# can-lehmann/exprgrad

Measured on AMD Instinct MI355X. Metric: GFLOP/s matmul 4096^3 f32 (1 GPU), higher is better.
Workload: dtype f32

## Files before the change

exprgrad_amd/csrc/kernels/gemm_f32_mfma.hip:

```cpp
#include "gemm_skinny.hpp"
#include "gemm_f32_pair.hpp"
#include "gemm_fused.hpp"
#include "gemm_layout.hpp"
#include "gemm_plan.hpp"

#include <algorithm>
#include <cstdio>
#include <cstdlib>
#include <cstring>
#include <string>
#include <type_traits>

#include "../eg_internal.hpp"

namespace {

using namespace eg::gemm;

inline bool aligned16(const void* p) { return (reinterpret_cast<uintptr_t>(p) & 15) == 0; }

const GemmSwitches& gemm_switches() {
  thread_local GemmSwitches s;
  thread_local unsigned seen = 0;
  const unsigned gen = eg::sw::generation();
// ... 119 lines not shown
  if (lane == 0) {
    float* c = C + m * ldc + n;
    float v = s;
    if (accumulate) v = *c + v;
    if (bias) v = v + bias[n];
    *c = v;
  }
}

__global__ __launch_bounds__(256) void gemm_small_kernel(const float* __restrict__ A, const float* __restrict__ B, float* C,
                                                         const float* __restrict__ bias, long M, long N, long K,
                                                         long a_sm, long a_sk, long b_sk, long b_sn, long ldc,
                                                         int accumulate) {
  gemm_small_body(blockIdx.x, A, B, C, bias, M, N, K, a_sm, a_sk, b_sk, b_sn, ldc, accumulate);
}

__global__ __launch_bounds__(256) void gemm_small_pair_kernel(eg::SmallGemm g0, eg::SmallGemm g1, long blocks0) {
  const bool second = (long)blockIdx.x >= blocks0;
  const eg::SmallGemm& g = second ? g1 : g0;
  gemm_small_body(second ? (long)blockIdx.x - blocks0 : (long)blockIdx.x, g.A, g.B, g.C, g.bias, g.M, g.N, g.K, g.a_sm, g.a_sk, g.b_sk,
                  g.b_sn, g.ldc, g.accumulate);
}

int run_gemm(eg_ctx* ctx, const GemmProblem& pr, GemmArgs args, const GemmSwitches& sw) {
  if (!args.ones_row) args.a_rows = args.M;
  const GemmPlan p = plan_gemm(pr, sw);
  const bool a_kc = pr.a_kc, b_kc = pr.b_kc;
  if (p.route == Route::Remainder) {
    for (int i = 0; i < p.nparts; ++i) {
      const auto& c = p.parts[i];
      GemmArgs part = args;
      part.A = args.A + c.row0 * (a_kc ? args.lda : 1);
      part.B = args.B + c.col0 * (b_kc ? args.ldb : 1);
      part.C = args.C + c.row0 * args.ldc + c.col0;
      if (args.bias) part.bias = args.bias + c.col0;
      part.M = part.a_rows = c.M;
      part.N = c.N;
      const int rc = run_gemm(ctx, problem_of(ctx, part, a_kc, b_kc, pr.conv, pr.vec_ok, pr.a_vec_only, true), part, sw);
      if (rc) return rc;
    }
    return EG_OK;
  }
  args.tiles_m = p.tiles_m;
  args.tiles_n = p.tiles_n;
  args.splits = p.splits;
  args.k_per_split = p.k_per_split;
  args.edge_splits = p.edge_splits;
  args.k_per_split_edge = p.k_per_split_edge;
  args.tail_tiles = p.tail_tiles;
  args.tail_splits = p.tail_splits;
  args.tail_k_per_split = p.tail_k_per_split;
  args.x_rows = p.x_rows;
  args.wide_store = p.wide_store;
  args.nt_store = p.nt_store;
  args.no_skew = p.no_skew;
  args.prio = p.prio && ctx->on_side_lane;
  float* scratch = nullptr;
  if (p.workspace_floats > 0) {
    const long scratch_floats = p.second == Second::Tree ? eg::colsum_scratch_floats(ctx, p.splits, args.M * args.N) : 0;
    const int rc = eg::ensure_workspace(ctx, (size_t)(p.workspace_floats + scratch_floats) * sizeof(float));
    if (rc) return rc;
    args.partial = static_cast<float*>(ctx->workspace);
    scratch = args.partial + p.workspace_floats;
  }
  const dim3 grid((unsigned)p.grid), block(p.block);
  const hipStream_t s = ctx->stream;
  switch (p.route) {
    case Route::Small:
      hipLaunchKernelGGL(gemm_small_kernel, grid, block, 0, s, args.A, args.B, args.C, args.bias, args.M, args.N, args.K,
                         a_kc ? args.lda : 1, a_kc ? 1 : args.lda, b_kc ? 1 : args.ldb, b_kc ? args.ldb : 1, args.ldc, args.accumulate);
      break;
    case Route::Skinny:
      hipLaunchKernelGGL((eg_skinny::gemm_skinny_nn_kernel<4>), grid, block, (size_t)args.K * 64, s, args.A, args.B, args.C, args.bias,
                         args.M, (int)args.N, (int)args.K, args.lda, args.ldb, args.ldc, args.accumulate);
      break;
    case Route::ExtraRows:
      if (sw.trace) args.trace = trace_begin(ctx, grid.x, 8);
      hipLaunchKernelGGL((gemm_f32_mfma_kernel<256, 256, BK, 128, 64, 1, false, false, 4, true, 0, 0, true, true>), grid, block, 0, s, args);
      EG_HIP_CHECK(hipGetLastError());
// ... 64 lines not shown

namespace eg {
namespace gemm {
const GemmSwitches& current_switches() { return gemm_switches(); }

int sgemm_exact(eg_ctx* ctx, int trans_a, int trans_b, long M, long N, long K, const float* A, long lda, const float* B, long ldb,
                float* C, long ldc, int accumulate, const float* bias, const unsigned* run_if, unsigned run_if_val) {
  EG_REQUIRE(ctx, EG_ERR_INVALID, "eg_sgemm: ctx is NULL");
  EG_REQUIRE(M >= 0 && N >= 0 && K >= 0, EG_ERR_INVALID, "eg_sgemm: negative extent");
  if (M == 0 || N == 0) return EG_OK;
  EG_REQUIRE(C, EG_ERR_INVALID, "eg_sgemm: C is NULL");
  EG_REQUIRE(K == 0 || (A && B), EG_ERR_INVALID, "eg_sgemm: NULL operand");
  EG_REQUIRE(lda >= (trans_a ? M : K) && ldb >= (trans_b ? K : N) && ldc >= N, EG_ERR_INVALID,
             "eg_sgemm: leading dimension smaller than the row length");
  int rc = eg::set_device(ctx);
  if (rc) return rc;

  GemmArgs args = sgemm_args(M, N, K, A, lda, B, ldb, C, ldc, accumulate, bias);
  args.run_if = run_if;
  args.run_if_val = run_if_val;
  return run_gemm(ctx, sgemm_problem(ctx, args, !trans_a, trans_b != 0), args, gemm_switches());
}

bool exact_single_launch(eg_ctx* ctx, int trans_a, int trans_b, long M, long N, long K, const float* A, long lda, const float* B,
                         long ldb, const float* C, long ldc, const float* bias) {
  const GemmArgs args = sgemm_args(M, N, K, A, lda, B, ldb, const_cast<float*>(C), ldc, 0, bias);
  return exact_single_launch(plan_gemm(sgemm_problem(ctx, args, !trans_a, trans_b != 0), gemm_switches()));
}
}
}

extern "C" int eg_sgemm(eg_ctx* ctx, int trans_a, int trans_b, int64_t M, int64_t N, int64_t K, const float* A,
                        int64_t lda, const float* B, int64_t ldb, float* C, int64_t ldc, int accumulate,
                        const float* bias) {
  const int rc = eg::gemm::sgemm_split(ctx, trans_a, trans_b, M, N, K, A, lda, B, ldb, C, ldc, accumulate, bias);
  if (rc != EG_ERR_UNSUPPORTED) return rc;
  return eg::gemm::sgemm_exact(ctx, trans_a, trans_b, M, N, K, A, lda, B, ldb, C, ldc, accumulate, bias);
}

namespace eg {
namespace gemm {
bool ones_row_supported(int trans_a, int trans_b, long M, long N, long K, const float* A, long lda, const float* B, long ldb) {
  const bool vec_a = operand_vec(lda, trans_a ? M : K, aligned16(A)), vec_b = operand_vec(ldb, trans_b ? K : N, aligned16(B));
  const char* off = eg::sw::raw("EG_NO_ONES_ROW");
  return vec_a && vec_b && K >= 16 && !((M + 1) * N <= 16384 && K <= 2048) && !(off && off[0] && off[0] != '0');
}

int sgemm_ones_row(eg_ctx* ctx, int trans_a, int trans_b, long M, long N, long K, const float* A, long lda, const float* B,
                   long ldb, float* C, long ldc, int accumulate) {
  EG_REQUIRE(ctx, EG_ERR_INVALID, "sgemm_ones_row: ctx is NULL");
// ... 402 lines not shown
```

exprgrad_amd/csrc/kernels/gemm_f32_mfma.hpp:

```cpp
#ifndef __HIPCC_RTC__
#pragma once
#include <hip/hip_runtime.h>
#endif

namespace eg {
namespace gemm {

typedef float f32x16 __attribute__((ext_vector_type(16)));
typedef float f32x4 __attribute__((ext_vector_type(4)));

struct GemmArgs {
  const float* A;
  const float* B;
  float* C;
  const float* bias;
  float* partial;
  long M, N, K;
  long lda, ldb, ldc;
  long k_per_split;
  int tiles_m, tiles_n;
  int accumulate;
  int splits;
  int edge_splits;
  long k_per_split_edge;
// ... 997 lines not shown
    const float* arow = park + (mb * 16 + r) * PS + 4 * g + kh * (BN / 2);
    const float* brow = w2s + ((g * 16 + r) << 2) + kh * (BN / 2) * 16;
    rd4 d0 = {0.f, 0.f, 0.f, 0.f}, d1 = {0.f, 0.f, 0.f, 0.f}, d2 = {0.f, 0.f, 0.f, 0.f}, d3 = {0.f, 0.f, 0.f, 0.f};
#pragma unroll
    for (int s2 = 0; s2 < BN / 32; s2 += 2) {
      const rd4 a0 = *reinterpret_cast<const rd4*>(arow + 16 * s2);
      const rd4 b0 = *reinterpret_cast<const rd4*>(brow + 256 * s2);
      const rd4 a1 = *reinterpret_cast<const rd4*>(arow + 16 * s2 + 16);
      const rd4 b1 = *reinterpret_cast<const rd4*>(brow + 256 * s2 + 256);
#pragma unroll
      for (int j = 0; j < 4; j += 2) {
        d0 = __builtin_amdgcn_mfma_f32_16x16x4f32(a0[j], b0[j], d0, 0, 0, 0);
        d1 = __builtin_amdgcn_mfma_f32_16x16x4f32(a1[j], b1[j], d1, 0, 0, 0);
        d2 = __builtin_amdgcn_mfma_f32_16x16x4f32(a0[j + 1], b0[j + 1], d2, 0, 0, 0);
        d3 = __builtin_amdgcn_mfma_f32_16x16x4f32(a1[j + 1], b1[j + 1], d3, 0, 0, 0);
      }
    }
#pragma unroll
    for (int v = 0; v < 4; ++v) half[v] = (d0[v] + d2[v]) + (d1[v] + d3[v]);
    if (kh == 1) *reinterpret_cast<rd4*>(rdx + (mb * 64 + lane) * 4) = rd4{half[0], half[1], half[2], half[3]};
  }
};

template <int BM, int BN, int BK, int WM, int WN, bool A_KC, bool B_KC, int VEC, bool EDGE, int CONV, int ABL, bool DMA,
          class Epi, bool XR = false>
__device__ __forceinline__ void gemm_block_at(const GemmArgs& a, const int block_id) {
  constexpr int WAVES = Geometry<BM, BN, WM, WN>::WAVES, WAVES_N = BN / WN;
  constexpr int MI = WM / 32, NI = WN / 32;
  constexpr int SA = LdsStride<BM, BK, A_KC>::value, SB = LdsStride<BN, BK, B_KC>::value;

  constexpr bool RD = Epi::RD_N > 0;
  constexpr int RD_FLOATS = RD ? 2 * (BM / WM) * 32 * (BN + 4) + BN * 16 + 4 * 64 * 4 : 0;
  constexpr int OPERAND_FLOATS = 2 * BK * (SA + SB) + (XR ? 2 * BK * 32 : 0);
  __shared__ __attribute__((aligned(16))) float lds[RD_FLOATS > OPERAND_FLOATS ? RD_FLOATS : OPERAND_FLOATS];

  const int tid = threadIdx.x;
  const int lane = tid & 63;
  const int wave = tid >> 6;
  const int wm0 = (wave / WAVES_N) * WM;
  const int wn0 = (wave % WAVES_N) * WN;
  if (a.run_if && *(volatile const unsigned*)a.run_if != a.run_if_val) return;
  if (a.prio) __builtin_amdgcn_s_setprio(3);
  trace_stamp<WAVES>(a, wave, lane, 0);

  const WorkItem w = decode_work<BM, BN>(a, block_id);
  const long m_blk = w.m_blk, n_blk = w.n_blk;
  const long k_begin = (long)w.split * w.k_slice;
  const long k_end = min(a.K, k_begin + w.k_slice);

  f32x16 acc[MI][NI];
  zero_acc(acc);
  if constexpr (RD) stage_row_product_weights<Epi, BM, BN, WM, WN>(a, lds, n_blk, tid);
  trace_stamp<WAVES>(a, wave, lane, 1);
  const bool il = run_k_loop<BM, BN, BK, WM, WN, A_KC, B_KC, VEC, EDGE, CONV, ABL, DMA, XR>(a, lds, acc, w, k_begin, k_end, tid, wm0, wn0);

  if constexpr ((ABL & 128) != 0) {
    float s = 0.f;
// ... 172 lines not shown
        }
      } else if (accumulate) {
#pragma unroll
        for (int r = 0; r < 16; ++r) {
          const long m = m_base + RS * acc_reg_row(r);
          if (m >= a.M || !n_ok) continue;
          col[m * ldo] = (col[m * ldo] + acc[i][j][r]) + bias;
        }
      } else {
#pragma unroll
        for (int r = 0; r < 16; ++r) {
          const long m = m_base + RS * acc_reg_row(r);
          if (m >= a.M || !n_ok) continue;
          col[m * ldo] = acc[i][j][r] + bias;
        }
      }
    }
  }
  trace_stamp<WAVES>(a, wave, lane, 3);
}

template <int BM, int BN, int BK, int WM, int WN, bool A_KC, bool B_KC, int VEC, bool EDGE, int CONV, int ABL, bool DMA,
          class Epi, bool XR = false>
__device__ __forceinline__ void gemm_block(const GemmArgs& a) {
  gemm_block_at<BM, BN, BK, WM, WN, A_KC, B_KC, VEC, EDGE, CONV, ABL, DMA, Epi, XR>(a, (int)blockIdx.x);
}

template <int BM, int BN, int WM, int WN, int MINB, bool EDGE, int VEC>
struct WavesPerSimd {
  static constexpr int plain = (MINB * Geometry<BM, BN, WM, WN>::WAVES + 3) / 4;
  static constexpr int value = (EDGE && VEC == 1 && BM * BN >= 128 * 64 && plain > 2) ? 2
                               : (EDGE && BN == 64 && BM >= 128 && plain == 4)        ? 3
                                                                                       : plain;
};

template <int BM, int BN, int BK, int WM, int WN, int MINB, bool A_KC, bool B_KC, int VEC, bool EDGE, int CONV,
          int ABL = 0, bool DMA = false, bool XR = false>
__global__ __launch_bounds__((Geometry<BM, BN, WM, WN>::NT), (WavesPerSimd<BM, BN, WM, WN, MINB, EDGE, VEC>::value)) void
gemm_f32_mfma_kernel(GemmArgs a) {
  gemm_block<BM, BN, BK, WM, WN, A_KC, B_KC, VEC, EDGE, CONV, ABL, DMA, EpiNone, XR>(a);
}

template <int BK, bool A_KC, bool B_KC>
__global__ __launch_bounds__(256, 4) void gemm_streamk_kernel(GemmArgs a) {
  constexpr int BM = 64, BN = 64, WM = 32, WN = 32;
  constexpr int SA = LdsStride<BM, BK, A_KC>::value, SB = LdsStride<BN, BK, B_KC>::value;
// ... 242 lines not shown
```

exprgrad_amd/csrc/kernels/gemm_fused.hpp:

```cpp
#pragma once
#include <string>

#include "../eg_internal.hpp"

namespace eg {
namespace gemm {

struct FusedLaunch {
  int bm = 0, bn = 0, bk = 0, wm = 0, wn = 0, minb = 0, nt = 0;
  bool a_kc = false, b_kc = false, edge = false, dma = false;
  int vec = 1;
  int splits = 1;
  unsigned grid = 0;
  bool narrow = false;
  int narrow_k = 0;
  unsigned narrow_grid = 0;
  long matrix_k_per_split = 0;
  alignas(8) unsigned char args[336];
  unsigned args_size = 0;
  unsigned waves = 0;
};
constexpr int MAX_EPILOGUE_OPERANDS = 6;

int plan_fused(eg_ctx* ctx, int trans_a, int trans_b, long M, long N, long K, const float* A, long lda, const float* B,
               long ldb, float* C, long ldc, const float* bias, FusedLaunch& out);

int sgemm_exact(eg_ctx* ctx, int trans_a, int trans_b, long M, long N, long K, const float* A, long lda, const float* B, long ldb,
                float* C, long ldc, int accumulate, const float* bias, const unsigned* run_if = nullptr, unsigned run_if_val = 0);
bool exact_single_launch(eg_ctx* ctx, int trans_a, int trans_b, long M, long N, long K, const float* A, long lda, const float* B,
                         long ldb, const float* C, long ldc, const float* bias);
int sgemm_split(eg_ctx* ctx, int trans_a, int trans_b, long M, long N, long K, const float* A, long lda, const float* B, long ldb,
                float* C, long ldc, int accumulate, const float* bias);

int sgemm_batched(eg_ctx* ctx, int trans_a, int trans_b, long batch, long M, long N, long K, const float* A, long lda, long stride_a,
                  const float* B, long ldb, long stride_b, float* C, long ldc, long stride_c, int accumulate, const float* bias);
int dgemm(eg_ctx* ctx, int trans_a, int trans_b, long M, long N, long K, const double* A, long lda, const double* B, long ldb, double* C,
          long ldc, int accumulate, const double* bias);
int dgemm_batched(eg_ctx* ctx, int trans_a, int trans_b, long batch, long M, long N, long K, const double* A, long lda, long stride_a,
                  const double* B, long ldb, long stride_b, double* C, long ldc, long stride_c, int accumulate, const double* bias);
struct GemmSwitches;
const GemmSwitches& current_switches();

bool ones_row_supported(int trans_a, int trans_b, long M, long N, long K, const float* A, long lda, const float* B, long ldb);
int sgemm_ones_row(eg_ctx* ctx, int trans_a, int trans_b, long M, long N, long K, const float* A, long lda, const float* B,
                   long ldb, float* C, long ldc, int accumulate);

void set_epilogue_operands(FusedLaunch& f, void* const* ptrs, int count, float grad_scale, long epoch);

void fused_withdraw_narrow(FusedLaunch& f);

bool fused_wide_store(const FusedLaunch& f);

std::string fused_variant(const FusedLaunch& f);
// ... 11 lines not shown
```

exprgrad_amd/csrc/kernels/gemm_plan.cpp:

```cpp
#include "gemm_plan.hpp"

#include <algorithm>
#include <cstdio>

namespace eg {
namespace gemm {

namespace {

struct TileCfg {
  int bm, bn, blocks_per_cu;
};

double ragged_tile_share(int bm, long m_rest) {
  const double live = (double)((m_rest + 31) / 32 * 32) / bm;
  const double floor = bm >= 256 ? 0.36 : 0.55;
  return live > floor ? live : floor;
}

double tile_cost(const TileCfg& t, long M, long N, long k_tiles, int cus, int& splits_out) {
  const long tm = (M + t.bm - 1) / t.bm, tn = (N + t.bn - 1) / t.bn;
  const long tiles = tm * tn;
  const long slots = (long)cus * t.blocks_per_cu;
  int splits = 1;
// ... 611 lines not shown
    long want = (CONV64_SLICE_BLOCKS_PER_CU * cus + r.grid_x - 1) / r.grid_x;
    want = std::min(want, std::min(r.K / CONV64_MIN_SLICE_PIXELS, 65535L));
    if (want > 1) {
      long per = (r.K + want - 1) / want;
      per = ((per + BK - 1) / BK) * BK;
      const long slices = (r.K + per - 1) / per;
      if (slices > 1) {
        r.slices = (int)slices;
        r.pixels_per_slice = per;
        r.workspace_doubles = slices * r.M * r.Ncols;
        r.reduce = true;
      }
    }
  }
  r.grid_y = r.slices;
  return r;
}

bool exact_single_launch(const GemmPlan& p) {
  return p.route == Route::Bk32 || (p.route == Route::Generic && p.bm == 256 && p.bn == 256 && !p.edge && p.splits <= 1 &&
                                    p.tail_tiles == 0 && p.second == Second::None);
}

}
}
```

exprgrad_amd/csrc/kernels/gemm_plan.hpp:

```cpp
#pragma once

namespace eg {
namespace gemm {

constexpr int BK = 16;

struct GemmProblem {
  long M = 0, N = 0, K = 0;
  bool a_kc = true, b_kc = false;
  long lda = 0, ldb = 0, ldc = 0;
  bool a_aligned = true, b_aligned = true, c_aligned = true;
  bool has_bias = false, bias_aligned = true;
  bool ones_row = false;
  int conv = 0;
  bool vec_ok = false, a_vec_only = false;
  bool piece = false;
  int cus = 256;
};

struct GemmSwitches {
  bool no_small = false, no_skinny = false;
  bool no_pair = false, no_t96 = false, no_streamk = false;
  bool no_xrow = false, no_bk32 = false, no_wide_store = false;
  bool no_skew = false, old_tile_model = false, small_bk32 = false;
// ... 138 lines not shown

constexpr long CONV64_MAX_INDEX = 1L << 31;

struct Conv64Plan {
  bool ok = false;
  long M = 0, Ncols = 0, K = 0;
  int config = 2;
  int bm = 0, bn = 0, wr = 0, wc = 0;
  bool vec_a = false, vec_b = false;
  int tiles_m = 0, tiles_n = 0;
  bool remap = false;
  long grid_x = 0, grid_y = 1;
  int slices = 1;
  long pixels_per_slice = 0;
  long workspace_doubles = 0;
  bool reduce = false;
  long aux_doubles = 0;
};

Conv64Plan plan_conv64(const Conv64Problem& p);

bool exact_single_launch(const GemmPlan& p);

}
}
```

exprgrad_amd/csrc/kernels/gemm_split_bf16.hip:

```cpp
#include <algorithm>
#include <cfloat>

#include "gemm_fused.hpp"
#include "../eg_internal.hpp"
#include "../switches.hpp"

namespace {

typedef __bf16 bf16x8 __attribute__((ext_vector_type(8)));
typedef __bf16 bf16x4 __attribute__((ext_vector_type(4)));
typedef float f32x4 __attribute__((ext_vector_type(4)));


struct SplitOperand {
  const float* src;
  long ld;
  long R;
  int kc;
  __bf16* dst;
};

__device__ __forceinline__ void unit_coords(const SplitOperand& o, long K, long u, long& r, long& chunk) {
  const long cpr = K / 8, t = u >> 6;
  const int l = (int)(u & 63);
  if (o.kc) {
    const long per = cpr / 4;
// ... 122 lines not shown
    *reinterpret_cast<bf16x4*>(row + c * 32 + 2 * IMG_PLANE) = h2;
  }
}

__device__ __forceinline__ int lane_unit(int lane) {
  const int quad = (lane >> 2) & 7;
  return ((lane >> 5) * 2 + (__builtin_popcount(quad) & 1)) * 16 + (quad >> 1) * 4 + (lane & 3);
}

__device__ __forceinline__ void store_tile(const SplitOperand& o, long K, long kt, long rb, const unsigned char* img) {
  const int wave = threadIdx.x >> 6, lane = threadIdx.x & 63;
  const long plane = o.R * K;
  __bf16* d = o.dst + (kt * o.R + rb * TILE_R) * 16;
#pragma unroll
  for (int p = 0; p < 3; ++p)
#pragma unroll
    for (int i = 0; i < 2; ++i) {
      const int u = (wave * 2 + i) * 64 + lane_unit(lane);
      const bf16x8 v = *reinterpret_cast<const bf16x8*>(img + p * IMG_PLANE + (u >> 4) * REC_BYTES + (u & 15) * 16);
      *reinterpret_cast<bf16x8*>(d + p * plane + u * 8) = v;
    }
}

__global__ __launch_bounds__(SPLIT_NT) void split_tiles_kernel(SplitOperand a, SplitOperand b, long K, int tiled, unsigned* flag,
                                                             unsigned epoch) {
  __shared__ __attribute__((aligned(16))) unsigned char img[2][IMG_BYTES];
  bool bad = false;
  int s = 0;
#pragma unroll
  for (int which = 0; which < 2; ++which) {
    const SplitOperand& o = which ? b : a;
    const long n = o.R * K / (TILE_R * 16);
    const long lo = n * blockIdx.x / gridDim.x, hi = n * (blockIdx.x + 1) / gridDim.x;
    if (!(tiled >> which & 1)) {
      const long units = o.R * K / 8;
      split_units<SPLIT_U>(o, o, K, units, lo * (SPLIT_NT * 2), hi * (SPLIT_NT * 2), bad);
      continue;
    }
    if (lo >= hi) continue;
    const long tr = o.R / TILE_R;
    long kt = lo / tr, rb = lo % tr;
    f32x4 x[4];
    load_tile(o, kt, rb, x);
    for (long t = lo; t < hi; ++t) {
      split_tile(x, img[s], bad);
      long nkt = kt, nrb = rb + 1;
      if (nrb == tr) {
        nrb = 0;
        ++nkt;
      }
      if (t + 1 < hi) load_tile(o, nkt, nrb, x);
      __syncthreads();
      store_tile(o, K, kt, rb, img[s]);
      s ^= 1;
      kt = nkt;
      rb = nrb;
    }
// ... 41 lines not shown
  const unsigned long v = reinterpret_cast<unsigned long>(p);
  const unsigned lo = __builtin_amdgcn_readfirstlane((unsigned)v), hi = __builtin_amdgcn_readfirstlane((unsigned)(v >> 32));
  return reinterpret_cast<const void*>(((unsigned long)hi << 32) | lo);
}

constexpr int ROLE_LOAD_OWN = 1, ROLE_LOAD_PARTNER = 2, ROLE_READ_TOP = 4, ROLE_READ_AHEAD = 8;
constexpr int PARTNER = 4;

#ifdef EG_SPLIT_GEMM_STAMPS
constexpr int STAMP_BLOCKS = 1024;
__device__ unsigned long long g_split_stamps[STAMP_BLOCKS][8][4];
#define EG_STAMP(t)                                                                  \
  do {                                                                               \
    __builtin_amdgcn_sched_barrier(0);                                               \
    asm volatile("s_memtime %0\n\ts_waitcnt lgkmcnt(0)" : "=s"(t)::"memory"); \
    __builtin_amdgcn_sched_barrier(0);                                               \
  } while (0)
#else
#define EG_STAMP(t) \
  do {              \
  } while (0)
#endif

__global__ __launch_bounds__(NT) void split_gemm_kernel(SplitGemmArgs a) {
  if (*(volatile const unsigned*)a.flag == a.epoch) return;
  __shared__ __attribute__((aligned(16))) unsigned char lds[STAGES * STAGE_BYTES];

  const int tid = threadIdx.x, lane = tid & 63, wave = __builtin_amdgcn_readfirstlane(tid >> 6);
  const int wr = wave >> 2, wc = wave & 3;
  long m_blk, n_blk;
  tile_origin(xcd_remap(blockIdx.x, gridDim.x), a.tiles_m, a.tiles_n, m_blk, n_blk);

  const __amdgpu_buffer_rsrc_t ra = __builtin_amdgcn_make_buffer_rsrc(
      const_cast<void*>(uniform_ptr(a.pa + m_blk * 16)), (short)0, -1, 0x00020000);
  const __amdgpu_buffer_rsrc_t rb = __builtin_amdgcn_make_buffer_rsrc(
      const_cast<void*>(uniform_ptr(a.pb + n_blk * 16)), (short)0, -1, 0x00020000);
  const unsigned a_plane = (unsigned)(a.M * a.K * 2), b_plane = (unsigned)(a.N * a.K * 2);
  const unsigned a_ktile = (unsigned)(a.M * 32), b_ktile = (unsigned)(a.N * 32);
  const unsigned voff = (unsigned)lane * 16;

  auto pieces = [&](int kt, int s, int w) {
    unsigned char* st = lds + s * STAGE_BYTES + w * 1024;
    const unsigned at = (unsigned)kt * a_ktile + (unsigned)w * 1024, bt = (unsigned)kt * b_ktile + (unsigned)w * 1024;
#pragma unroll
    for (int i = 0; i < LOADS; ++i) {
      __attribute__((address_space(3))) void* dst = (__attribute__((address_space(3))) void*)(st + i * PLANE_BYTES);
      if (i < 3)
        __builtin_amdgcn_raw_ptr_buffer_load_lds(ra, dst, 16, voff, (unsigned)i * a_plane + at, 0, 0);
      else
        __builtin_amdgcn_raw_ptr_buffer_load_lds(rb, dst, 16, voff, (unsigned)(i - 3) * b_plane + bt, 0, 0);
// ... 110 lines not shown
  if (a.bias) b4 = *reinterpret_cast<const f32x4*>(a.bias + col);
#pragma unroll
  for (int h = 0; h < 2; ++h) {
#pragma unroll
    for (int i = 0; i < 4; ++i)
#pragma unroll
      for (int j = 0; j < 4; ++j)
#pragma unroll
        for (int r = 0; r < 4; ++r) park[(i * 16 + 4 * prow + r) * WN + j * 16 + (lane & 15)] = acc[4 * h + i][j][r];
    asm volatile("s_waitcnt lgkmcnt(0)" ::: "memory");
#pragma unroll
    for (int q = 0; q < 16; ++q) {
      const int row = 4 * q + prow;
      f32x4 v = *reinterpret_cast<const f32x4*>(park + row * WN + pc4);
      f32x4* c = reinterpret_cast<f32x4*>(a.C + (m_blk + wr * WM + h * 64 + row) * a.ldc + col);
      if (a.accumulate) v = *c + v;
      if (a.bias) v = v + b4;
      *c = v;
    }
    asm volatile("s_waitcnt lgkmcnt(0)" ::: "memory");
  }
}

inline bool aligned16(const void* p) { return (reinterpret_cast<uintptr_t>(p) & 15) == 0; }

constexpr size_t kPlaneCap = 1ull << 30;

}

namespace eg {
namespace gemm {

int sgemm_split(eg_ctx* ctx, int trans_a, int trans_b, long M, long N, long K, const float* A, long lda, const float* B, long ldb,
                float* C, long ldc, int accumulate, const float* bias) {
  if (!ctx || !A || !B || !C || M <= 0 || N <= 0 || K <= 0) return EG_ERR_UNSUPPORTED;
  if (lda < (trans_a ? M : K) || ldb < (trans_b ? K : N) || ldc < N) return EG_ERR_UNSUPPORTED;
  if (eg::sw::on("EG_NO_SPLIT_GEMM")) return EG_ERR_UNSUPPORTED;
  if (M % BM != 0 || N % BN != 0 || K % 32 != 0 || K < 2048) return EG_ERR_UNSUPPORTED;
  if ((M / BM) * (N / BN) < ctx->compute_units) return EG_ERR_UNSUPPORTED;
  const size_t plane_bytes = 6 * (size_t)(M + N) * (size_t)K;
  if (plane_bytes > kPlaneCap || 6 * (size_t)std::max(M, N) * (size_t)K >= (1ull << 31)) return EG_ERR_UNSUPPORTED;
  if (!aligned16(A) || !aligned16(B) || (!trans_a && lda % 4 != 0) || (trans_b && ldb % 4 != 0)) return EG_ERR_UNSUPPORTED;
  if (!aligned16(C) || ldc % 4 != 0 || (bias && !aligned16(bias))) return EG_ERR_UNSUPPORTED;
  if (!exact_single_launch(ctx, trans_a, trans_b, M, N, K, A, lda, B, ldb, C, ldc, bias)) return EG_ERR_UNSUPPORTED;

  int rc = eg::set_device(ctx);
  if (rc) return rc;
  if (!ctx->split_flag) {
    EG_HIP_CHECK(hipMalloc((void**)&ctx->split_flag, sizeof(unsigned)));
    EG_HIP_CHECK(hipMemset(ctx->split_flag, 0, sizeof(unsigned)));
  }
  rc = eg::ensure_workspace(ctx, plane_bytes);
  if (rc) return rc;
  if (++ctx->split_epoch == 0) ctx->split_epoch = 1;
  const unsigned epoch = ctx->split_epoch;

  __bf16* pa = static_cast<__bf16*>(ctx->workspace);
  __bf16* pb = pa + 3 * (size_t)M * K;
  const SplitOperand oa = {A, lda, M, trans_a ? 0 : 1, pa};
  const SplitOperand ob = {B, ldb, N, trans_b ? 1 : 0, pb};
  const bool scalar = eg::sw::on("EG_SPLIT_PASS_SCALAR");
  const int tiled = (!scalar && !oa.kc && lda % 4 == 0 ? 1 : 0) | (!scalar && !ob.kc && ldb % 4 == 0 ? 2 : 0);
  if (tiled) {
    const long blocks = (long)TILE_BLOCKS_PER_CU * ctx->compute_units;
    hipLaunchKernelGGL(split_tiles_kernel, dim3((unsigned)blocks), dim3(SPLIT_NT), 0, ctx->stream, oa, ob, K, tiled, ctx->split_flag,
                       epoch);
  } else {
    const long units_a = M * K / 8, units = (M + N) * K / 8;
    long blocks = (units + SPLIT_NT * SPLIT_U - 1) / (SPLIT_NT * SPLIT_U);
    if (blocks > 8L * ctx->compute_units) blocks = 8L * ctx->compute_units;
    hipLaunchKernelGGL(split_planes_kernel, dim3((unsigned)blocks), dim3(SPLIT_NT), 0, ctx->stream, oa, ob, K, units_a, units,
                       ctx->split_flag, epoch);
  }
  EG_HIP_CHECK(hipGetLastError());

  SplitGemmArgs g = {};
  g.pa = pa;
  g.pb = pb;
  g.C = C;
  g.bias = bias;
  g.M = M;
  g.N = N;
  g.K = K;
  g.ldc = ldc;
  g.tiles_m = (int)(M / BM);
  g.tiles_n = (int)(N / BN);
  g.accumulate = accumulate;
  g.skew = eg::sw::present("EG_GEMM_NO_SKEW") ? 0 : 1;
  g.flag = ctx->split_flag;
  g.epoch = epoch;
  hipLaunchKernelGGL(split_gemm_kernel, dim3((unsigned)(g.tiles_m * g.tiles_n)), dim3(NT), 0, ctx->stream, g);
  EG_HIP_CHECK(hipGetLastError());

  return sgemm_exact(ctx, trans_a, trans_b, M, N, K, A, lda, B, ldb, C, ldc, accumulate, bias, ctx->split_flag, epoch);
}

}
}

#ifdef EG_SPLIT_GEMM_STAMPS
extern "C" int eg_debug_split_stamps(unsigned long long* dst, size_t count) {
  if (count > sizeof(g_split_stamps) / sizeof(unsigned long long)) return EG_ERR_UNSUPPORTED;
  EG_HIP_CHECK(hipDeviceSynchronize());
  EG_HIP_CHECK(hipMemcpyFromSymbol(dst, HIP_SYMBOL(g_split_stamps), count * sizeof(unsigned long long)));
  return 0;
}
#endif
```

exprgrad_amd/csrc/switches.cpp:

```cpp
#include "switches.hpp"

#include <cstdio>
#include <cstring>
#include <mutex>
#include <string>
#include <unordered_map>
#include <vector>

#include "exprgrad_hip.h"

namespace {

struct Row {
  const char* name;
  const char* cls;
  const char* purpose;
};

const Row kSwitches[] = {
    {"EG_TUNING", "execution", "honour the rows of class `tuning` (measurement aids); unset: they are ignored"},
    {"EG_NO_GRAPH", "execution", "launch one by one instead of replaying captured HIP graphs"},
    {"EG_NO_DPP_BUTTERFLY", "execution", "row groups exchange lanes through the LDS crossbar in every step of a wave reduction (no DPP moves)"},
    {"EG_NO_DEFERRED_FOLD", "execution", "a row group in front of a side-lane group folds its partial rows itself, not on the side lane"},
    {"EG_NO_OVERLAP", "execution", "no side lane: bandwidth-bound launches run in front of the long contraction, not next to it"},
// ... 2 lines not shown
    {"EG_NO_INLINE", "execution", "no producer / consumer inlining of elementwise kernels into generated kernels"},
    {"EG_NO_ALIAS", "execution", "whole-tensor raw copies (reshape) are copied instead of sharing storage"},
    {"EG_NO_ONES_ROW", "execution", "bias gradient as its own column sum instead of the weight gradient's virtual row of ones"},
    {"EG_NO_SMALL_GEMM", "execution", "tiny contractions on the matrix tiles instead of one wave per output element"},
    {"EG_NO_NARROW_INDEX", "execution", "64-bit index arithmetic everywhere in generated kernels"},
    {"EG_NO_PREDICATE", "execution", "pre-activations stored as values, not as predicate bits"},
    {"EG_NO_ROW_PRODUCT", "execution", "the 10-wide forward product as its own launch, not in the previous layer's epilogue"},
    {"EG_NO_ROW_DIRECT", "execution", "a one-block row group writes a partial row for row_finalize instead of its totals"},
    {"EG_NO_BATCHED_GEMM", "execution", "products with a leading batch index as generated kernels instead of eg_bgemm launches / collapsed products"},
    {"EG_NO_SMALL_PAIR", "execution", "two independent tiny contractions as two launches"},
    {"EG_NO_SKINNY_GEMM", "execution", "N <= 16 products on the matrix tiles instead of the streaming skinny kernel"},
    {"EG_NO_NARROW_K", "execution", "K <= 16 products with a generated epilogue on the matrix tile instead of the streaming kernel"},
    {"EG_NO_SAMPLE_FUSE", "execution", "no sample groups (one block per sample): the launch chain of a small-batch step"},
    {"EG_OVERLAP_SIDE_FIRST", "execution", "the side lane's launches are issued in front of the long contraction they run beside (the order of rounds 2 - 5)"},
    {"EG_SAMPLE_KEEP_BARRIERS", "execution", "sample kernels keep the barrier between independent members"},
    {"EG_SAMPLE_NO_STAGE", "execution", "a sample group's members read parameters from global memory, not from a copy in LDS"},
    {"EG_SAMPLE_NO_MFMA", "execution", "convolution members of a sample group as scalar loop nests, not on the matrix cores"},
    {"EG_NO_SLAB_FOLD", "execution", "the optimizer's map group does not add up the sample kernel's slab rows itself"},
    {"EG_NO_SLAB_SUM", "execution", "k-slices folded by the two-launch column sum instead of slab_sum"},
    {"EG_NO_ROW_TAIL", "execution", "a row group's last block neither folds the partial rows nor runs the update"},
    {"EG_PIPELINE", "execution", "the batch pipeline (two half batches, streaming launches under the other half's contraction): OFF unless 1"},
    {"EG_NO_SPLIT_GEMM", "execution", "eg_sgemm runs every product on the exact f32 matrix path, never as three-way split bf16"},
    {"EG_SPLIT_PASS_SCALAR", "execution", "the split pass reads an operand whose k runs along ld as 4-byte loads per lane (units), not as 16-byte tiles through LDS"},
    {"EG_GEMM_NO_SKEW", "execution", "every wave of a contraction block runs the k loop in phase (the round-3 loop)"},
    {"EG_GEMM_NO_BK32", "execution", "16-deep k-tiles for long whole-tile products"},
    {"EG_GEMM_NO_PAIR", "execution", "no wave-pair / eight-wave small-tile kernels"},
    {"EG_GEMM_NO_T96", "execution", "no 96 x 96 whole-round tiles"},
    {"EG_GEMM_NO_STREAMK", "execution", "64 x 64 tiles one block per tile, not persistent stream-K blocks"},
    {"EG_GEMM_NO_XROW", "execution", "1 .. 32 rows beyond whole tiles as a ragged tile row, not a ninth accumulator block"},
    {"EG_GEMM_NO_WIDE_STORE", "execution", "tiles leave as 128-byte pieces instead of through LDS as whole rows"},
    {"EG_CONV_NO_TINY", "execution", "small convolutions on the contraction route"},
    {"EG_CONV_NO_GRADF_HALO", "execution", "filter gradient as one gathered contraction"},
    {"EG_CONV_NO_WIDE_STORE", "execution", "halo convolution stores 128-byte pieces"},
    {"EG_CONV_NO_VIRTUAL_PAD", "execution", "image gradient reads a padded copy of the output gradient"},
    {"EG_CONV_NO_HALO", "execution", "3 x 3-class convolutions on the implicit-GEMM route"},
    {"EG_CONV_NO_DIRECT", "execution", "few-channel convolutions on the implicit-GEMM route"},
    {"EG_CONV_NO_BAND", "execution", "small-channel convolutions on the routes the band kernels replaced"},
    {"EG_CONV_NO_MFMA64", "execution", "float64 convolutions that the band and direct kernels decline: generated kernels in a model, refused by the eg_conv2_nhwc*_f64 entry points"},
    {"EG_NO_STAGED_COPY", "execution", "downloads into pageable memory as one runtime copy"},
    {"EG_FIT_NO_DIRECT", "execution", "fit copies every batch into the inputs' staging buffers"},
    {"EG_DP_REAGREE_STEPS", "data-parallel", "steps between two negotiations of the exchange schedule (default 256; 0: only the first)"},
    {"EG_DP_INIT_TIMEOUT_S", "data-parallel", "watchdog on ncclCommInitRank, seconds (default 180)"},
    {"EG_DP_RESERVE_CUS", "data-parallel", "compute units the tail range leaves to RCCL's kernel (default 8)"},
    {"EG_DP_TEST_AS_MULTI", "data-parallel", "a one-rank group takes the N > 1 code paths (one-GPU boxes)"},
    {"EG_DP_NO_SPLIT", "data-parallel", "groups start with the early / late split of the bucket forbidden (eg_dp_set_split)"},
    {"EG_HIPRTC_LIB", "compiler", "path of the libhiprtc the library opens"},
// ... 121 lines not shown
```

Before: 256,100.

## Merge split-bf16 product with exact fallback; add banded split pass

The split-bf16 product kernel and its exact f32 fallback are merged into one kernel that reads the flag once and runs one body or the other in shared LDS. This removes a launch per GEMM. The split pass also gains a banded form for k-contiguous operands: each wave reads 1 KiB row segments with nontemporal loads, converts them into three bf16 planes in LDS, and stores them with the next band's load overlapped. The costs are more template instantiations and sharing the LDS budget between the two GEMM bodies.

```diff
diff --git a/exprgrad_amd/csrc/kernels/gemm_f32_mfma.hip b/exprgrad_amd/csrc/kernels/gemm_f32_mfma.hip
--- a/exprgrad_amd/csrc/kernels/gemm_f32_mfma.hip
+++ b/exprgrad_amd/csrc/kernels/gemm_f32_mfma.hip
@@ -165,6 +165,23 @@
                   g.b_sn, g.ldc, g.accumulate);
 }
 
+void set_plan_args(const eg_ctx* ctx, const GemmPlan& p, GemmArgs& args) {
+  args.tiles_m = p.tiles_m;
+  args.tiles_n = p.tiles_n;
+  args.splits = p.splits;
+  args.k_per_split = p.k_per_split;
+  args.edge_splits = p.edge_splits;
+  args.k_per_split_edge = p.k_per_split_edge;
+  args.tail_tiles = p.tail_tiles;
+  args.tail_splits = p.tail_splits;
+  args.tail_k_per_split = p.tail_k_per_split;
+  args.x_rows = p.x_rows;
+  args.wide_store = p.wide_store;
+  args.nt_store = p.nt_store;
+  args.no_skew = p.no_skew;
+  args.prio = p.prio && ctx->on_side_lane;
+}
+
 int run_gemm(eg_ctx* ctx, const GemmProblem& pr, GemmArgs args, const GemmSwitches& sw) {
   if (!args.ones_row) args.a_rows = args.M;
   const GemmPlan p = plan_gemm(pr, sw);
@@ -184,20 +201,7 @@
     }
     return EG_OK;
   }
-  args.tiles_m = p.tiles_m;
-  args.tiles_n = p.tiles_n;
-  args.splits = p.splits;
-  args.k_per_split = p.k_per_split;
-  args.edge_splits = p.edge_splits;
-  args.k_per_split_edge = p.k_per_split_edge;
-  args.tail_tiles = p.tail_tiles;
-  args.tail_splits = p.tail_splits;
-  args.tail_k_per_split = p.tail_k_per_split;
-  args.x_rows = p.x_rows;
-  args.wide_store = p.wide_store;
-  args.nt_store = p.nt_store;
-  args.no_skew = p.no_skew;
-  args.prio = p.prio && ctx->on_side_lane;
+  set_plan_args(ctx, p, args);
   float* scratch = nullptr;
   if (p.workspace_floats > 0) {
     const long scratch_floats = p.second == Second::Tree ? eg::colsum_scratch_floats(ctx, p.splits, args.M * args.N) : 0;
@@ -308,10 +312,13 @@
   return run_gemm(ctx, sgemm_problem(ctx, args, !trans_a, trans_b != 0), args, gemm_switches());
 }
 
-bool exact_single_launch(eg_ctx* ctx, int trans_a, int trans_b, long M, long N, long K, const float* A, long lda, const float* B,
-                         long ldb, const float* C, long ldc, const float* bias) {
-  const GemmArgs args = sgemm_args(M, N, K, A, lda, B, ldb, const_cast<float*>(C), ldc, 0, bias);
-  return exact_single_launch(plan_gemm(sgemm_problem(ctx, args, !trans_a, trans_b != 0), gemm_switches()));
+GemmPlan exact_plan(eg_ctx* ctx, int trans_a, int trans_b, long M, long N, long K, const float* A, long lda, const float* B, long ldb,
+                    float* C, long ldc, int accumulate, const float* bias, GemmArgs& args) {
+  args = sgemm_args(M, N, K, A, lda, B, ldb, C, ldc, accumulate, bias);
+  args.a_rows = M;
+  const GemmPlan p = plan_gemm(sgemm_problem(ctx, args, !trans_a, trans_b != 0), gemm_switches());
+  if (p.route == Route::Bk32) set_plan_args(ctx, p, args);
+  return p;
 }
 }
 }
diff --git a/exprgrad_amd/csrc/kernels/gemm_f32_mfma.hpp b/exprgrad_amd/csrc/kernels/gemm_f32_mfma.hpp
--- a/exprgrad_amd/csrc/kernels/gemm_f32_mfma.hpp
+++ b/exprgrad_amd/csrc/kernels/gemm_f32_mfma.hpp
@@ -1043,17 +1043,21 @@
   }
 };
 
+template <int BM, int BN, int BK, int WM, bool A_KC, bool B_KC, class Epi, bool XR>
+struct BlockLds {
+  static constexpr int SA = LdsStride<BM, BK, A_KC>::value, SB = LdsStride<BN, BK, B_KC>::value;
+  static constexpr int RD_FLOATS = Epi::RD_N > 0 ? 2 * (BM / WM) * 32 * (BN + 4) + BN * 16 + 4 * 64 * 4 : 0;
+  static constexpr int OPERAND_FLOATS = 2 * BK * (SA + SB) + (XR ? 2 * BK * 32 : 0);
+  static constexpr int FLOATS = RD_FLOATS > OPERAND_FLOATS ? RD_FLOATS : OPERAND_FLOATS;
+};
+
 template <int BM, int BN, int BK, int WM, int WN, bool A_KC, bool B_KC, int VEC, bool EDGE, int CONV, int ABL, bool DMA,
           class Epi, bool XR = false>
-__device__ __forceinline__ void gemm_block_at(const GemmArgs& a, const int block_id) {
+__device__ __forceinline__ void gemm_block_body(const GemmArgs& a, const int block_id, float* lds) {
   constexpr int WAVES = Geometry<BM, BN, WM, WN>::WAVES, WAVES_N = BN / WN;
   constexpr int MI = WM / 32, NI = WN / 32;
   constexpr int SA = LdsStride<BM, BK, A_KC>::value, SB = LdsStride<BN, BK, B_KC>::value;
-
   constexpr bool RD = Epi::RD_N > 0;
-  constexpr int RD_FLOATS = RD ? 2 * (BM / WM) * 32 * (BN + 4) + BN * 16 + 4 * 64 * 4 : 0;
-  constexpr int OPERAND_FLOATS = 2 * BK * (SA + SB) + (XR ? 2 * BK * 32 : 0);
-  __shared__ __attribute__((aligned(16))) float lds[RD_FLOATS > OPERAND_FLOATS ? RD_FLOATS : OPERAND_FLOATS];
 
   const int tid = threadIdx.x;
   const int lane = tid & 63;
@@ -1272,6 +1276,13 @@
 
 template <int BM, int BN, int BK, int WM, int WN, bool A_KC, bool B_KC, int VEC, bool EDGE, int CONV, int ABL, bool DMA,
           class Epi, bool XR = false>
+__device__ __forceinline__ void gemm_block_at(const GemmArgs& a, const int block_id) {
+  __shared__ __attribute__((aligned(16))) float lds[BlockLds<BM, BN, BK, WM, A_KC, B_KC, Epi, XR>::FLOATS];
+  gemm_block_body<BM, BN, BK, WM, WN, A_KC, B_KC, VEC, EDGE, CONV, ABL, DMA, Epi, XR>(a, block_id, lds);
+}
+
+template <int BM, int BN, int BK, int WM, int WN, bool A_KC, bool B_KC, int VEC, bool EDGE, int CONV, int ABL, bool DMA,
+          class Epi, bool XR = false>
 __device__ __forceinline__ void gemm_block(const GemmArgs& a) {
   gemm_block_at<BM, BN, BK, WM, WN, A_KC, B_KC, VEC, EDGE, CONV, ABL, DMA, Epi, XR>(a, (int)blockIdx.x);
 }
diff --git a/exprgrad_amd/csrc/kernels/gemm_fused.hpp b/exprgrad_amd/csrc/kernels/gemm_fused.hpp
--- a/exprgrad_amd/csrc/kernels/gemm_fused.hpp
+++ b/exprgrad_amd/csrc/kernels/gemm_fused.hpp
@@ -27,8 +27,10 @@
 
 int sgemm_exact(eg_ctx* ctx, int trans_a, int trans_b, long M, long N, long K, const float* A, long lda, const float* B, long ldb,
                 float* C, long ldc, int accumulate, const float* bias, const unsigned* run_if = nullptr, unsigned run_if_val = 0);
-bool exact_single_launch(eg_ctx* ctx, int trans_a, int trans_b, long M, long N, long K, const float* A, long lda, const float* B,
-                         long ldb, const float* C, long ldc, const float* bias);
+struct GemmArgs;
+struct GemmPlan;
+GemmPlan exact_plan(eg_ctx* ctx, int trans_a, int trans_b, long M, long N, long K, const float* A, long lda, const float* B, long ldb,
+                    float* C, long ldc, int accumulate, const float* bias, GemmArgs& args);
 int sgemm_split(eg_ctx* ctx, int trans_a, int trans_b, long M, long N, long K, const float* A, long lda, const float* B, long ldb,
                 float* C, long ldc, int accumulate, const float* bias);
 
diff --git a/exprgrad_amd/csrc/kernels/gemm_plan.cpp b/exprgrad_amd/csrc/kernels/gemm_plan.cpp
--- a/exprgrad_amd/csrc/kernels/gemm_plan.cpp
+++ b/exprgrad_amd/csrc/kernels/gemm_plan.cpp
@@ -657,5 +657,12 @@
                                     p.tail_tiles == 0 && p.second == Second::None);
 }
 
-}
-}
+SplitLaunchPlan plan_split_launches(const GemmPlan& exact, bool separate_fallback) {
+  SplitLaunchPlan r;
+  r.merged = exact.route == Route::Bk32 && !separate_fallback;
+  r.launches = r.merged ? 2 : 3;
+  return r;
+}
+
+}
+}
diff --git a/exprgrad_amd/csrc/kernels/gemm_plan.hpp b/exprgrad_amd/csrc/kernels/gemm_plan.hpp
--- a/exprgrad_amd/csrc/kernels/gemm_plan.hpp
+++ b/exprgrad_amd/csrc/kernels/gemm_plan.hpp
@@ -184,5 +184,11 @@
 
 bool exact_single_launch(const GemmPlan& p);
 
+struct SplitLaunchPlan {
+  int launches = 3;
+  bool merged = false;
+};
+SplitLaunchPlan plan_split_launches(const GemmPlan& exact, bool separate_fallback);
+
 }
 }
diff --git a/exprgrad_amd/csrc/kernels/gemm_split_bf16.hip b/exprgrad_amd/csrc/kernels/gemm_split_bf16.hip
--- a/exprgrad_amd/csrc/kernels/gemm_split_bf16.hip
+++ b/exprgrad_amd/csrc/kernels/gemm_split_bf16.hip
@@ -1,7 +1,9 @@
 #include <algorithm>
 #include <cfloat>
 
+#include "gemm_f32_mfma.hpp"
 #include "gemm_fused.hpp"
+#include "gemm_plan.hpp"
 #include "../eg_internal.hpp"
 #include "../switches.hpp"
 
@@ -170,8 +172,60 @@
     }
 }
 
-__global__ __launch_bounds__(SPLIT_NT) void split_tiles_kernel(SplitOperand a, SplitOperand b, long K, int tiled, unsigned* flag,
-                                                             unsigned epoch) {
+constexpr int BAND_R = 32, BAND_K = 256;
+constexpr int BAND_KT_BYTES = BAND_R * 32 + 32;
+constexpr int BAND_PLANE = (BAND_K / 16) * BAND_KT_BYTES;
+static_assert(3 * BAND_PLANE <= 2 * IMG_BYTES, "a band's image fits the two tile images");
+static_assert(BAND_R * BAND_K == 2 * TILE_R * 16, "a band is two tiles' worth: a block's run of tiles is a run of bands");
+
+__device__ __forceinline__ void load_band(const SplitOperand& o, long rb, long ks, f32x4 (&x)[8]) {
+  const int wave = __builtin_amdgcn_readfirstlane(threadIdx.x >> 6), lane = threadIdx.x & 63;
+  const float* p = o.src + (rb * BAND_R + wave * 8) * o.ld + ks * BAND_K + lane * 4;
+#pragma unroll
+  for (int i = 0; i < 8; ++i) x[i] = __builtin_nontemporal_load(reinterpret_cast<const f32x4*>(p + i * o.ld));
+}
+
+__device__ __forceinline__ void split_band(const f32x4 (&x)[8], unsigned char* img, bool& bad) {
+  const int wave = __builtin_amdgcn_readfirstlane(threadIdx.x >> 6), lane = threadIdx.x & 63;
+  unsigned char* piece = img + (lane >> 2) * BAND_KT_BYTES + wave * 8 * 32 + (lane & 3) * 8;
+#pragma unroll
+  for (int i = 0; i < 8; ++i) {
+    bf16x4 h0, h1, h2;
+#pragma unroll
+    for (int c = 0; c < 4; ++c) {
+      __bf16 b0, b1, b2;
+      split_elem(x[i][c], b0, b1, b2, bad);
+      h0[c] = b0;
+      h1[c] = b1;
+      h2[c] = b2;
+    }
+    *reinterpret_cast<bf16x4*>(piece + i * 32) = h0;
+    *reinterpret_cast<bf16x4*>(piece + i * 32 + BAND_PLANE) = h1;
+    *reinterpret_cast<bf16x4*>(piece + i * 32 + 2 * BAND_PLANE) = h2;
+    __builtin_amdgcn_sched_barrier(0);
+  }
+}
+
+__device__ __forceinline__ void store_band(const SplitOperand& o, long K, long rb, long ks, const unsigned char* img) {
+  const int wave = __builtin_amdgcn_readfirstlane(threadIdx.x >> 6), lane = threadIdx.x & 63;
+  const long plane = o.R * K;
+  const unsigned char* src = img + wave * 4 * BAND_KT_BYTES + lane * 16;
+  __bf16* d = o.dst + ((ks * (BAND_K / 16) + wave * 4) * o.R + rb * BAND_R) * 16 + lane * 8;
+#pragma unroll
+  for (int p = 0; p < 3; ++p) {
+#pragma unroll
+    for (int j = 0; j < 4; ++j) {
+      const bf16x8 v = *reinterpret_cast<const bf16x8*>(src + p * BAND_PLANE + j * BAND_KT_BYTES);
+      *reinterpret_cast<bf16x8*>(d + p * plane + j * o.R * 16) = v;
+    }
+  }
+}
+
+constexpr int PASS_UNITS = 0, PASS_TILES = 1, PASS_BANDS = 2;
+
+template <int FORM_A, int FORM_B>
+__global__ __launch_bounds__(SPLIT_NT, TILE_BLOCKS_PER_CU) void split_tiles_kernel(SplitOperand a, SplitOperand b, long K, unsigned* flag,
+                                                                                 unsigned epoch) {
   __shared__ __attribute__((aligned(16))) unsigned char img[2][IMG_BYTES];
   bool bad = false;
   int s = 0;
@@ -180,7 +234,32 @@
     const SplitOperand& o = which ? b : a;
     const long n = o.R * K / (TILE_R * 16);
     const long lo = n * blockIdx.x / gridDim.x, hi = n * (blockIdx.x + 1) / gridDim.x;
-    if (!(tiled >> which & 1)) {
+    const int form = which ? FORM_B : FORM_A;
+    if (form == PASS_BANDS) {
+      const long n2 = n / 2, lo2 = n2 * blockIdx.x / gridDim.x, hi2 = n2 * (blockIdx.x + 1) / gridDim.x;
+      if (lo2 >= hi2) continue;
+      const int kb = (int)(K / BAND_K);
+      int rb = __builtin_amdgcn_readfirstlane((int)(lo2 / kb)), ks = __builtin_amdgcn_readfirstlane((int)(lo2 % kb));
+      f32x4 x[8];
+      load_band(o, rb, ks, x);
+      for (long t = lo2; t < hi2; ++t) {
+        __syncthreads();
+        split_band(x, &img[0][0], bad);
+        int nrb = rb, nks = ks + 1;
+        if (nks == kb) {
+          nks = 0;
+          ++nrb;
+        }
+        if (t + 1 < hi2) load_band(o, nrb, nks, x);
+        __syncthreads();
+        store_band(o, K, rb, ks, &img[0][0]);
+        rb = nrb;
+        ks = nks;
+      }
+      __syncthreads();
+      continue;
+    }
+    if (form == PASS_UNITS) {
       const long units = o.R * K / 8;
       split_units<SPLIT_U>(o, o, K, units, lo * (SPLIT_NT * 2), hi * (SPLIT_NT * 2), bad);
       continue;
@@ -268,10 +347,7 @@
   } while (0)
 #endif
 
-__global__ __launch_bounds__(NT) void split_gemm_kernel(SplitGemmArgs a) {
-  if (*(volatile const unsigned*)a.flag == a.epoch) return;
-  __shared__ __attribute__((aligned(16))) unsigned char lds[STAGES * STAGE_BYTES];
-
+__device__ __forceinline__ void split_product_body(const SplitGemmArgs a, unsigned char* lds) {
   const int tid = threadIdx.x, lane = tid & 63, wave = __builtin_amdgcn_readfirstlane(tid >> 6);
   const int wr = wave >> 2, wc = wave & 3;
   long m_blk, n_blk;
@@ -428,6 +504,30 @@
   }
 }
 
+__device__ __forceinline__ unsigned read_flag(const unsigned* flag) {
+  return __builtin_amdgcn_readfirstlane(*(volatile const unsigned*)flag);
+}
+
+__global__ __launch_bounds__(NT) void split_gemm_kernel(SplitGemmArgs a) {
+  if (*(volatile const unsigned*)a.flag == a.epoch) return;
+  __shared__ __attribute__((aligned(16))) unsigned char lds[STAGES * STAGE_BYTES];
+  split_product_body(a, lds);
+}
+
+template <bool AKC, bool BKC>
+using ExactLds = eg::gemm::BlockLds<BM, BN, 32, WM, AKC, BKC, eg::gemm::EpiNone, false>;
+
+template <bool AKC, bool BKC>
+__global__ __launch_bounds__(NT) void sgemm_split_or_exact_kernel(SplitGemmArgs a, eg::gemm::GemmArgs x) {
+  static_assert(ExactLds<AKC, BKC>::FLOATS * sizeof(float) <= STAGES * STAGE_BYTES, "the exact tile body fits the product's stages");
+  __shared__ __attribute__((aligned(16))) unsigned char lds[STAGES * STAGE_BYTES];
+  if (read_flag(a.flag) != a.epoch)
+    split_product_body(a, lds);
+  else
+    eg::gemm::gemm_block_body<BM, BN, 32, WM, WN, AKC, BKC, 4, false, 0, 0, true, eg::gemm::EpiNone>(x, (int)blockIdx.x,
+                                                                                                    reinterpret_cast<float*>(lds));
+}
+
 inline bool aligned16(const void* p) { return (reinterpret_cast<uintptr_t>(p) & 15) == 0; }
 
 constexpr size_t kPlaneCap = 1ull << 30;
@@ -448,7 +548,10 @@
   if (plane_bytes > kPlaneCap || 6 * (size_t)std::max(M, N) * (size_t)K >= (1ull << 31)) return EG_ERR_UNSUPPORTED;
   if (!aligned16(A) || !aligned16(B) || (!trans_a && lda % 4 != 0) || (trans_b && ldb % 4 != 0)) return EG_ERR_UNSUPPORTED;
   if (!aligned16(C) || ldc % 4 != 0 || (bias && !aligned16(bias))) return EG_ERR_UNSUPPORTED;
-  if (!exact_single_launch(ctx, trans_a, trans_b, M, N, K, A, lda, B, ldb, C, ldc, bias)) return EG_ERR_UNSUPPORTED;
+  GemmArgs exact_args;
+  const GemmPlan exact = exact_plan(ctx, trans_a, trans_b, M, N, K, A, lda, B, ldb, C, ldc, accumulate, bias, exact_args);
+  if (!exact_single_launch(exact)) return EG_ERR_UNSUPPORTED;
+  const SplitLaunchPlan launches = plan_split_launches(exact, eg::sw::on("EG_SPLIT_SEPARATE_FALLBACK"));
 
   int rc = eg::set_device(ctx);
   if (rc) return rc;
@@ -467,10 +570,23 @@
   const SplitOperand ob = {B, ldb, N, trans_b ? 1 : 0, pb};
   const bool scalar = eg::sw::on("EG_SPLIT_PASS_SCALAR");
   const int tiled = (!scalar && !oa.kc && lda % 4 == 0 ? 1 : 0) | (!scalar && !ob.kc && ldb % 4 == 0 ? 2 : 0);
-  if (tiled) {
+  const bool bands = !eg::sw::on("EG_SPLIT_PASS_UNITS") && K % BAND_K == 0;
+  const int banded = (bands && oa.kc ? 1 : 0) | (bands && ob.kc ? 2 : 0);
+  if (tiled | banded) {
     const long blocks = (long)TILE_BLOCKS_PER_CU * ctx->compute_units;
-    hipLaunchKernelGGL(split_tiles_kernel, dim3((unsigned)blocks), dim3(SPLIT_NT), 0, ctx->stream, oa, ob, K, tiled, ctx->split_flag,
-                       epoch);
+    const int form_a = banded & 1 ? PASS_BANDS : tiled & 1 ? PASS_TILES : PASS_UNITS;
+    const int form_b = banded & 2 ? PASS_BANDS : tiled & 2 ? PASS_TILES : PASS_UNITS;
+    auto launch = [&](auto kernel) {
+      hipLaunchKernelGGL(kernel, dim3((unsigned)blocks), dim3(SPLIT_NT), 0, ctx->stream, oa, ob, K, ctx->split_flag, epoch);
+    };
+    if (form_a == PASS_BANDS && form_b == PASS_TILES) launch(split_tiles_kernel<PASS_BANDS, PASS_TILES>);
+    else if (form_a == PASS_BANDS && form_b == PASS_BANDS) launch(split_tiles_kernel<PASS_BANDS, PASS_BANDS>);
+    else if (form_a == PASS_TILES && form_b == PASS_TILES) launch(split_tiles_kernel<PASS_TILES, PASS_TILES>);
+    else if (form_a == PASS_TILES && form_b == PASS_BANDS) launch(split_tiles_kernel<PASS_TILES, PASS_BANDS>);
+    else if (form_a == PASS_BANDS) launch(split_tiles_kernel<PASS_BANDS, PASS_UNITS>);
+    else if (form_b == PASS_BANDS) launch(split_tiles_kernel<PASS_UNITS, PASS_BANDS>);
+    else if (form_a == PASS_TILES) launch(split_tiles_kernel<PASS_TILES, PASS_UNITS>);
+    else launch(split_tiles_kernel<PASS_UNITS, PASS_TILES>);
   } else {
     const long units_a = M * K / 8, units = (M + N) * K / 8;
     long blocks = (units + SPLIT_NT * SPLIT_U - 1) / (SPLIT_NT * SPLIT_U);
@@ -495,7 +611,16 @@
   g.skew = eg::sw::present("EG_GEMM_NO_SKEW") ? 0 : 1;
   g.flag = ctx->split_flag;
   g.epoch = epoch;
-  hipLaunchKernelGGL(split_gemm_kernel, dim3((unsigned)(g.tiles_m * g.tiles_n)), dim3(NT), 0, ctx->stream, g);
+  const dim3 grid((unsigned)(g.tiles_m * g.tiles_n));
+  if (launches.merged) {
+    if (trans_a && trans_b) hipLaunchKernelGGL((sgemm_split_or_exact_kernel<false, true>), grid, dim3(NT), 0, ctx->stream, g, exact_args);
+    else if (trans_a) hipLaunchKernelGGL((sgemm_split_or_exact_kernel<false, false>), grid, dim3(NT), 0, ctx->stream, g, exact_args);
+    else if (trans_b) hipLaunchKernelGGL((sgemm_split_or_exact_kernel<true, true>), grid, dim3(NT), 0, ctx->stream, g, exact_args);
+    else hipLaunchKernelGGL((sgemm_split_or_exact_kernel<true, false>), grid, dim3(NT), 0, ctx->stream, g, exact_args);
+    EG_HIP_CHECK(hipGetLastError());
+    return EG_OK;
+  }
+  hipLaunchKernelGGL(split_gemm_kernel, grid, dim3(NT), 0, ctx->stream, g);
   EG_HIP_CHECK(hipGetLastError());
 
   return sgemm_exact(ctx, trans_a, trans_b, M, N, K, A, lda, B, ldb, C, ldc, accumulate, bias, ctx->split_flag, epoch);
diff --git a/exprgrad_amd/csrc/switches.cpp b/exprgrad_amd/csrc/switches.cpp
--- a/exprgrad_amd/csrc/switches.cpp
+++ b/exprgrad_amd/csrc/switches.cpp
@@ -48,6 +48,8 @@
     {"EG_PIPELINE", "execution", "the batch pipeline (two half batches, streaming launches under the other half's contraction): OFF unless 1"},
     {"EG_NO_SPLIT_GEMM", "execution", "eg_sgemm runs every product on the exact f32 matrix path, never as three-way split bf16"},
     {"EG_SPLIT_PASS_SCALAR", "execution", "the split pass reads an operand whose k runs along ld as 4-byte loads per lane (units), not as 16-byte tiles through LDS"},
+    {"EG_SPLIT_PASS_UNITS", "execution", "the split pass reads a k-contiguous operand in units of 8 k (2 x 16 bytes per lane), not as 1 KiB row segments through LDS"},
+    {"EG_SPLIT_SEPARATE_FALLBACK", "execution", "the split-bf16 product and its exact fallback as two launches behind the split pass, not as one kernel that runs either"},
     {"EG_GEMM_NO_SKEW", "execution", "every wave of a contraction block runs the k loop in phase (the round-3 loop)"},
     {"EG_GEMM_NO_BK32", "execution", "16-deep k-tiles for long whole-tile products"},
     {"EG_GEMM_NO_PAIR", "execution", "no wave-pair / eight-wave small-tile kernels"},
```

Result: no change. 258,600 (median of 6 runs) (+1.0%).
